# mwhittaker/frankenpaxos

Hardware: NVIDIA H100
Metric: committed slots/sec (simulated) at 1M in-flight slots (higher is better)
Workload: dtype int32

## Files before the change

frankenpaxos_b200/_lib.py:

```python
import ctypes as C
import os

from . import build as _build

_lib = None

SYMBOLS = [
    "fpx_abi_version", "fpx_strerror", "fpx_last_error", "fpx_create", "fpx_destroy", "fpx_reset",
    "fpx_proxyleader_arm", "fpx_acceptor_phase2a", "fpx_proxyleader_phase2b", "fpx_replica_chosen",
    "fpx_chosen_watermark", "fpx_quorum_eval", "fpx_snapshot_acceptor", "fpx_snapshot_log",
    "fpx_proxyleader_arm_dev", "fpx_acceptor_phase2a_dev", "fpx_proxyleader_phase2b_dev",
    "fpx_replica_chosen_dev", "fpx_replica_chosen_last_dev", "fpx_chosen_watermark_dev", "fpx_sync",
    "fpx_stream", "fpx_launch_count", "fpx_set_coop_ctas_per_sm", "fpx_step_dev", "fpx_step_kernel_ms", "fpx_step_arm_ms",
    "fpx_acceptor_phase1a", "fpx_leader_safe_values",
    "fpx_vm_client_request", "fpx_vm_phase2a", "fpx_vm_learn_chosen", "fpx_vm_skip", "fpx_vm_client_request_dev", "fpx_vm_phase2a_dev", "fpx_vm_step_dev",
    "fpx_mencius_arm_range", "fpx_mencius_acceptor_noop_range", "fpx_mencius_range_phase2b",
    "fpx_mencius_replica_chosen_range", "fpx_mencius_replica_range_first", "fpx_mencius_replica_range_fill",
    "fpx_wire_decode_inbound", "fpx_wire_decode_inbound_dev", "fpx_wire_encode_phase2b", "fpx_wire_encode_phase2b_dev",
    "fpx_wire_encode_nack", "fpx_wire_encode_chosen",
    "fpx_step_submit", "fpx_step_wait", "fpx_retire_below", "fpx_exchange_export", "fpx_exchange_attach", "fpx_exchange_attach_local", "fpx_exchange_epoch",
    "fpx_global_watermark", "fpx_global_watermark_dev",
    "fpx_conflict_index_create", "fpx_conflict_index_destroy", "fpx_conflict_index_put_snapshot", "fpx_conflict_index_batch",
    "fpx_depgraph_create", "fpx_depgraph_destroy", "fpx_depgraph_commit", "fpx_depgraph_update_executed", "fpx_depgraph_execute",
    "fpx_epaxos_stream", "fpx_epaxos_sync", "fpx_epaxos_lead_dev", "fpx_epaxos_preaccept_dev", "fpx_epaxos_accept_dev",
# ... 47 lines not shown
    L.fpx_snapshot_acceptor.restype = i32
    L.fpx_snapshot_log.argtypes = [vp, i32, i32, vp]; L.fpx_snapshot_log.restype = i32
    L.fpx_proxyleader_arm_dev.argtypes = [vp, vp, i32]; L.fpx_proxyleader_arm_dev.restype = i32
    L.fpx_acceptor_phase2a_dev.argtypes = [vp, vp, i32, vp, vp]; L.fpx_acceptor_phase2a_dev.restype = i32
    L.fpx_proxyleader_phase2b_dev.argtypes = [vp, vp, i32, vp]; L.fpx_proxyleader_phase2b_dev.restype = i32
    L.fpx_replica_chosen_dev.argtypes = [vp, vp, i32]; L.fpx_replica_chosen_dev.restype = i32
    L.fpx_replica_chosen_last_dev.argtypes = [vp, vp]; L.fpx_replica_chosen_last_dev.restype = i32
    L.fpx_chosen_watermark_dev.argtypes = [vp, vp]; L.fpx_chosen_watermark_dev.restype = i32
    L.fpx_acceptor_phase1a.argtypes = [vp, i32, i32, i32, p(i32)]; L.fpx_acceptor_phase1a.restype = i32
    L.fpx_leader_safe_values.argtypes = [vp, C.c_uint32, i32, i32, vp, vp, p(i32)]; L.fpx_leader_safe_values.restype = i32
    L.fpx_vm_client_request.argtypes = [vp, vp, i32, p(i64)]; L.fpx_vm_client_request.restype = i32
    L.fpx_vm_phase2a.argtypes = [vp, vp, i32, vp, p(i64)]; L.fpx_vm_phase2a.restype = i32
    L.fpx_vm_learn_chosen.argtypes = [vp, vp, i32, p(i64)]; L.fpx_vm_learn_chosen.restype = i32
    L.fpx_vm_skip.argtypes = [vp, vp, i32, p(i64)]; L.fpx_vm_skip.restype = i32
    L.fpx_vm_client_request_dev.argtypes = [vp, vp, i32]; L.fpx_vm_client_request_dev.restype = i32
    L.fpx_vm_phase2a_dev.argtypes = [vp, vp, i32, vp]; L.fpx_vm_phase2a_dev.restype = i32
    L.fpx_mencius_arm_range.argtypes = [vp, vp, i32, p(i64)]; L.fpx_mencius_arm_range.restype = i32
    L.fpx_mencius_acceptor_noop_range.argtypes = [vp, vp, i32, vp, p(i32), vp, p(i32), p(i64)]
    L.fpx_mencius_acceptor_noop_range.restype = i32
    L.fpx_mencius_range_phase2b.argtypes = [vp, vp, i32, vp, p(i32), p(i64)]; L.fpx_mencius_range_phase2b.restype = i32
    L.fpx_mencius_replica_chosen_range.argtypes = [vp, vp, i32, p(i64)]
    L.fpx_mencius_replica_chosen_range.restype = i32
    L.fpx_mencius_replica_range_first.argtypes = [vp, vp, i32, vp, p(i64)]; L.fpx_mencius_replica_range_first.restype = i32
    L.fpx_mencius_replica_range_fill.argtypes = [vp, vp, i32, vp, p(i64)]; L.fpx_mencius_replica_range_fill.restype = i32
    L.fpx_wire_decode_inbound.argtypes = [vp, i32, vp, vp, i32, vp, vp, p(i64)]; L.fpx_wire_decode_inbound.restype = i32
    L.fpx_wire_decode_inbound_dev.argtypes = [vp, i32, vp, vp, i32, vp, vp]; L.fpx_wire_decode_inbound_dev.restype = i32
    L.fpx_wire_encode_phase2b.argtypes = [vp, vp, i32, vp, i32, vp, p(i64)]; L.fpx_wire_encode_phase2b.restype = i32
    L.fpx_wire_encode_phase2b_dev.argtypes = [vp, vp, i32, vp, i32, vp]; L.fpx_wire_encode_phase2b_dev.restype = i32
    L.fpx_wire_encode_nack.argtypes = [vp, vp, i32, vp, i32, vp, p(i64)]; L.fpx_wire_encode_nack.restype = i32
    L.fpx_wire_encode_chosen.argtypes = [vp, vp, i32, vp, vp, i32, vp, i32, vp, p(i64)]
    L.fpx_wire_encode_chosen.restype = i32
    L.fpx_step_dev.argtypes = [vp, vp, i32, vp, i32, vp, vp, vp, i32, vp, vp, i32]; L.fpx_step_dev.restype = i32
    L.fpx_vm_step_dev.argtypes = [vp, vp, i32, vp, i32, vp, vp, i32, vp, vp]; L.fpx_vm_step_dev.restype = i32
    L.fpx_step_kernel_ms.argtypes = [vp, i32, p(C.c_float), p(C.c_float)]; L.fpx_step_kernel_ms.restype = i32
    L.fpx_step_arm_ms.argtypes = [vp, i32, p(C.c_float)]; L.fpx_step_arm_ms.restype = i32
    L.fpx_sync.argtypes = [vp, p(SyncResult)]; L.fpx_sync.restype = i32
    L.fpx_set_coop_ctas_per_sm.argtypes = [vp, i32]; L.fpx_set_coop_ctas_per_sm.restype = i32
    L.fpx_stream.argtypes = [vp]; L.fpx_stream.restype = vp
    L.fpx_launch_count.argtypes = [vp]; L.fpx_launch_count.restype = i64
    L.fpx_retire_below.argtypes = [vp, i32]; L.fpx_retire_below.restype = i32
    L.fpx_step_submit.argtypes = [vp, vp, i32, vp, i32, vp, i32, vp, vp, vp]; L.fpx_step_submit.restype = i32
    L.fpx_step_wait.argtypes = [vp, p(i32), p(i32), p(i32), p(i32), p(i64)]; L.fpx_step_wait.restype = i32
    L.fpx_exchange_export.argtypes = [vp, vp]; L.fpx_exchange_export.restype = i32
    L.fpx_exchange_attach.argtypes = [vp, i32, vp]; L.fpx_exchange_attach.restype = i32
    L.fpx_exchange_attach_local.argtypes = [vp, i32, vp]; L.fpx_exchange_attach_local.restype = i32
    L.fpx_exchange_epoch.argtypes = [vp]; L.fpx_exchange_epoch.restype = C.c_uint32
    L.fpx_global_watermark_dev.argtypes = [vp, C.c_uint32, i32, vp, vp]; L.fpx_global_watermark_dev.restype = i32
    L.fpx_global_watermark.argtypes = [vp, C.c_uint32, i32, p(i32), vp]; L.fpx_global_watermark.restype = i32
    if hasattr(L, "fpx_debug_set_tally_path"):
        L.fpx_debug_set_tally_path.argtypes = [vp, i32]; L.fpx_debug_set_tally_path.restype = i32
        L.fpx_debug_last_tally_path.argtypes = [vp]; L.fpx_debug_last_tally_path.restype = i32
    if hasattr(L, "fpx_debug_set_acceptor_segments"):
        L.fpx_debug_set_acceptor_segments.argtypes = [vp, i32]; L.fpx_debug_set_acceptor_segments.restype = i32
    if L.fpx_abi_version() != 1:
        raise ImportError("libfpx.so ABI version mismatch")
    _lib = L
    return L
```

frankenpaxos_b200/csrc/fpx_arm.cuh:

```cuda
#pragma once
#include "fpx_common.cuh"
#include "fpx_ranges.cuh"

namespace fpx {

struct ArmConflict { int32_t slot, round; };

struct ArmParams {
  Geometry g;
  PLState pl;
  const int4* in;
  int32_t n;
  DevStatus* st;
  ArmConflict* conflicts;
  uint32_t* win_bits;
  unsigned long long* votes;
  int32_t vanilla;
  RangeTable rng;
  int32_t check_rng;
};

__device__ __forceinline__ void note_arm_conflict(const ArmParams& P, int slot, int round) {
  uint32_t c = atomicAdd(&P.st->n_arm_conflicts, 1u);
  if (c < (uint32_t)kMaxConflicts) P.conflicts[c] = ArmConflict{slot, round};
}

__device__ __forceinline__ bool claim_header(const ArmParams& P, RowRef r, int slot, int round, int value,
                                             bool* other_round) {
  unsigned long long want = ((unsigned long long)(uint32_t)value << 32) | (uint32_t)round;
  unsigned long long old = atomicCAS(r.hdr64(), kU64Empty, want);
  *other_round = false;
  if (old == kU64Empty) return true;
  uint32_t orw = (uint32_t)old;
  if ((int)(orw & ~kDoneBit) != round) { *other_round = true; return false; }
  if ((uint32_t)(old >> 32) != (uint32_t)value) note_arm_conflict(P, slot, round);
  return false;
}

__device__ __forceinline__ uint32_t* table_insert(const ArmParams& P, int slot, int round) {
  const Geometry& g = P.g;
  if (g.ovf_cap == 0) return nullptr;
  unsigned long long key = ((unsigned long long)(uint32_t)slot << 32) | (uint32_t)round;
  uint32_t h = (uint32_t)mix64(key) & g.ovf_mask;
  for (int probe = 0; probe < g.ovf_cap; ++probe) {
    unsigned long long k = atomicCAS(&P.pl.ovf_keys[h], kU64Empty, key);
    if (k == kU64Empty || k == key) return P.pl.ovf_rows + (size_t)h * g.row_words;
    h = (h + 1) & g.ovf_mask;
  }
  return nullptr;
}

__device__ __forceinline__ bool arm_finish(const ArmParams& P, const int4& rec, unsigned long long old, int i) {
  const Geometry& g = P.g;
  const int slot = rec.x, round = rec.y, value = rec.z;
  if (old == kU64Empty) return true;
  uint32_t* prim = P.pl.rows + (size_t)local_slot(g, slot) * g.row_words;
  unsigned long long* hdr = (unsigned long long*)prim;
  while (true) {
    uint32_t orw = (uint32_t)old;
    if (orw == kBusy) {
      __nanosleep(64);
      old = *(volatile unsigned long long*)hdr;
      continue;
    }
    if (orw == kPoison) {
      uint32_t* t = table_insert(P, slot, round);
      if (t == nullptr) { report_error(P.st, FPX_ERR_OVERFLOW_FULL, i); return false; }
      bool dummy;
      return claim_header(P, RowRef{t}, slot, round, value, &dummy);
    }
    if ((int)(orw & ~kDoneBit) == round) {
      if ((uint32_t)(old >> 32) != (uint32_t)value) note_arm_conflict(P, slot, round);
      return false;
// ... 73 lines not shown
      if (local[u] >= 0 && old[u] != kU64Empty) {
        const int4 rec = __ldcg(P.in + i);
        won = arm_finish(P, rec, old[u], i);
        self = rec.w & 0xffff;
      } else if (won && P.vanilla) {
        self = rel_to_slot(g, ring_to_rel(g, local[u])) % g.per_group;
      }
      if (won && P.vanilla) {
        uint32_t* row = P.pl.rows + (size_t)local[u] * g.row_words;
        auto stamp = [&](int w) { return w - 2 == self ? 0u : kStampEmpty; };
        *(uint2*)(row + 2) = make_uint2(stamp(2), stamp(3));
        for (int w = 4; w < g.row_words; w += 4) *(uint4*)(row + w) = make_uint4(stamp(w), stamp(w + 1), stamp(w + 2), stamp(w + 3));
        red_max_u64(&P.votes[cell_index(g, local[u], self)], (((want[u] & 0xffffffffull) + 1ull) << 32) | (want[u] >> 32));
      }
      unsigned wb = __ballot_sync(0xffffffffu, won);
      if (lane == 0) P.win_bits[c0 + u] = wb;
      int ml = __reduce_max_sync(0xffffffffu, won ? local[u] : -1);
      if (lane == 0 && ml > max_local) max_local = ml;
    }
  }
  return max_local;
}

__device__ __forceinline__ void arm_resolve_conflicts(const ArmParams& P) {
  const Geometry& g = P.g;
  __shared__ int s_min, s_any;
  uint32_t nc = __ldcg(&P.st->n_arm_conflicts);
  if (nc == 0) return;
  if (nc > (uint32_t)kMaxConflicts) {
    if (threadIdx.x == 0) { report_error(P.st, FPX_ERR_CONFLICT, 0); P.st->n_arm_conflicts = 0; }
    return;
  }
  for (uint32_t c = 0; c < nc; ++c) {
    int slot = P.conflicts[c].slot, round = P.conflicts[c].round;
    if (threadIdx.x == 0) { s_min = INT_MAX; s_any = 0; }
    __syncthreads();
    for (int j = threadIdx.x; j < P.n; j += blockDim.x) {
      int4 rec = P.in[j];
      if (rec.x == slot && rec.y == round) {
        atomicMin(&s_min, j);
        if ((__ldcg(&P.win_bits[j >> 5]) >> (j & 31)) & 1u) s_any = 1;
      }
    }
    __syncthreads();
    if (threadIdx.x == 0 && s_any && s_min != INT_MAX) {
      RowRef r = find_row(g, P.pl, local_slot(g, slot), slot, round);
      if (r.p != nullptr) r.p[1] = (uint32_t)P.in[s_min].z;
    }
    __syncthreads();
  }
  if (threadIdx.x == 0) P.st->n_arm_conflicts = 0;
}

__global__ void __launch_bounds__(kArmThreads, 1) arm_kernel(ArmParams P) {
  const int lane = threadIdx.x & 31;
  const int max_local = arm_chunks(P, blockIdx.x * (blockDim.x >> 5) + (threadIdx.x >> 5), gridDim.x * (blockDim.x >> 5), lane);
  if (lane == 0 && max_local >= 0) atomicMax(&P.st->max_armed_local, max_local);

  __shared__ bool s_last;
  __syncthreads();
  if (threadIdx.x == 0) {
    __threadfence();
    s_last = (atomicAdd(&P.st->ticket, 1u) == gridDim.x - 1);
  }
  __syncthreads();
  if (!s_last) return;
  __threadfence();
  if (threadIdx.x == 0) P.st->ticket = 0;
  arm_resolve_conflicts(P);
}

}
```

frankenpaxos_b200/csrc/fpx_common.cuh:

```cuda
#pragma once
#include <cuda_runtime.h>
#include <stdint.h>

#include "../../include/fpx.h"

namespace fpx {

constexpr uint32_t kUnarmed = 0xffffffffu;
constexpr uint32_t kDoneBit = 0x80000000u;
constexpr uint32_t kPoison = 0xfffffffeu;
constexpr uint32_t kBusy = 0xfffffffdu;
constexpr uint32_t kStampEmpty = 0xffffffffu;
constexpr uint64_t kU64Empty = ~0ull;
constexpr uint64_t kCellChosen = 0x8000000000000000ull;
constexpr int kThreads = 256;
constexpr int kWarps = kThreads / 32;
constexpr int kMaxKeys = FPX_MAX_ACCEPTORS;
constexpr int kMaxConflicts = 1024;
constexpr int kSms = 132;
constexpr int kMaxGrid = kSms * 8;
constexpr uint32_t kTsBadVoter = 1u, kTsAnomaly = 2u, kTsPoison = 4u, kTsVanillaRound = 8u;

struct DevStatus {
  unsigned long long err_word;
  int32_t n_p2b, n_nack, n_chosen, watermark;
  uint32_t n_conflicts;
  uint32_t ticket;
  int32_t wm_local;
  int32_t max_chosen_local;
  int32_t wm_found;
  uint32_t bar_count;
  uint32_t nack_total;
  uint32_t pad[2];
  int32_t max_armed_local;
  uint32_t bar_gen;
  int32_t ts_min_local, ts_max_local;
  int32_t ts_min_round, ts_max_round;
  uint32_t ts_flags;
  uint32_t ts_path;
  uint32_t n_arm_conflicts;
  uint32_t wm_need_scan;
  unsigned long long t_acceptor[8];
  unsigned long long t_tally[8];
};

__device__ __forceinline__ unsigned long long global_timer_ns() {
  unsigned long long t;
  asm volatile("mov.u64 %0, %%globaltimer;" : "=l"(t));
  return t;
}
#define FPX_MARK(arr, k) do { if (blockIdx.x == 0 && threadIdx.x == 0) (arr)[k] = global_timer_ns(); } while (0)

constexpr int kMaxShards = 64;
struct DevExchange {
  int32_t enabled, n, mine, pad;
  uint32_t epoch;
  uint32_t pad2;
  unsigned long long* tabs[kMaxShards];
};
__device__ __forceinline__ void exchange_publish(DevExchange* x, int global_frontier) {
  if (x == nullptr || !x->enabled) return;
  const uint32_t ep = ++x->epoch;
  const unsigned long long v = ((unsigned long long)ep << 32) | (uint32_t)global_frontier;
  for (int p = 0; p < x->n; ++p)
    if (x->tabs[p] != nullptr)
      asm volatile("st.global.relaxed.sys.u64 [%0], %1;" ::"l"(x->tabs[p] + x->mine), "l"(v) : "memory");
}

struct Geometry {
  int32_t protocol, f, groups, per_group, flexible, num_leaders;
  int32_t voters;
  int32_t num_keys;
  int32_t quorum;
  int32_t row_words;
  int32_t slot_capacity;
  int32_t local_slots;
  int32_t base_local;
  int32_t base_ring;
  int32_t shard_index, shard_count;
  uint32_t ovf_mask;
  int32_t ovf_cap;
  unsigned long long m_groups, m_shards;
  int32_t cell_shift;
  int32_t lgroups, agroups;
  unsigned long long m_lgroups, m_agroups;
};

__device__ __forceinline__ uint32_t fastmod_u32(uint32_t a, unsigned long long M, uint32_t d) {
  unsigned long long low = M * a;
  return (uint32_t)__umul64hi(low, d);
}
__device__ __forceinline__ uint32_t fastdiv_u32(uint32_t a, unsigned long long M) {
  return (uint32_t)__umul64hi(M, a);
}

__device__ __forceinline__ int4 ld_stream(const int4* p) {
  int4 r;
  asm volatile("ld.global.nc.L1::no_allocate.v4.s32 {%0,%1,%2,%3}, [%4];"
               : "=r"(r.x), "=r"(r.y), "=r"(r.z), "=r"(r.w)
               : "l"(p));
  return r;
}
__device__ __forceinline__ unsigned long long l2_policy_evict_last() {
  unsigned long long pol;
  asm volatile("createpolicy.fractional.L2::evict_last.b64 %0, 1.0;" : "=l"(pol));
  return pol;
}
__device__ __forceinline__ unsigned long long l2_policy_evict_normal() {
  unsigned long long pol;
  asm volatile("createpolicy.fractional.L2::evict_normal.b64 %0, 1.0;" : "=l"(pol));
  return pol;
}
__device__ __forceinline__ unsigned long long l2_policy_evict_first() {
  unsigned long long pol;
  asm volatile("createpolicy.fractional.L2::evict_first.b64 %0, 1.0;" : "=l"(pol));
  return pol;
}
__device__ __forceinline__ void st_evict_first(int4* p, int4 v, unsigned long long pol) {
  asm volatile("st.global.L1::no_allocate.L2::cache_hint.v4.s32 [%0], {%1,%2,%3,%4}, %5;" ::"l"(p), "r"(v.x), "r"(v.y),
               "r"(v.z), "r"(v.w), "l"(pol));
}
__device__ __forceinline__ int4 ld_keep(const int4* p, unsigned long long pol) {
  int4 r;
  asm volatile("ld.global.nc.L1::no_allocate.L2::cache_hint.v4.s32 {%0,%1,%2,%3}, [%4], %5;"
               : "=r"(r.x), "=r"(r.y), "=r"(r.z), "=r"(r.w)
               : "l"(p), "l"(pol));
  return r;
}
__device__ __forceinline__ int4 ld_hint(const int4* p, unsigned long long pol) {
  int4 r;
  asm volatile("ld.global.L1::no_allocate.L2::cache_hint.v4.s32 {%0,%1,%2,%3}, [%4], %5;"
               : "=r"(r.x), "=r"(r.y), "=r"(r.z), "=r"(r.w)
               : "l"(p), "l"(pol));
  return r;
}
__device__ __forceinline__ unsigned long long ld_u64_evict_last(const unsigned long long* p) {
  unsigned long long v;
  asm volatile("{ .reg .b64 pol; createpolicy.fractional.L2::evict_last.b64 pol, 1.0; "
               "ld.global.cg.L2::cache_hint.u64 %0, [%1], pol; }"
               : "=l"(v) : "l"(p));
  return v;
}

__device__ __forceinline__ void red_min_u32(uint32_t* p, uint32_t v) {
  asm volatile("red.global.min.u32 [%0], %1;" ::"l"(p), "r"(v) : "memory");
}
__device__ __forceinline__ void red_or_u32(uint32_t* p, uint32_t v) {
  asm volatile("red.global.or.b32 [%0], %1;" ::"l"(p), "r"(v) : "memory");
}
__device__ __forceinline__ void red_min_u64(unsigned long long* p, unsigned long long v) {
  asm volatile("red.global.min.u64 [%0], %1;" ::"l"(p), "l"(v) : "memory");
}
__device__ __forceinline__ void red_max_u64(unsigned long long* p, unsigned long long v) {
  asm volatile("red.global.max.u64 [%0], %1;" ::"l"(p), "l"(v) : "memory");
}
__device__ __forceinline__ void st_stream(int4* p, int4 v) {
  asm volatile("st.global.L1::no_allocate.v4.s32 [%0], {%1,%2,%3,%4};" ::"l"(p), "r"(v.x), "r"(v.y),
               "r"(v.z), "r"(v.w));
}
__device__ __forceinline__ void st_stream2(int2* p, int2 v) {
  asm volatile("st.global.L1::no_allocate.v2.s32 [%0], {%1,%2};" ::"l"(p), "r"(v.x), "r"(v.y));
}
__device__ __forceinline__ unsigned lanemask_lt() {
  unsigned m;
  asm("mov.u32 %0, %%lanemask_lt;" : "=r"(m));
  return m;
}

__device__ __forceinline__ void report_error(DevStatus* st, int code, long long index) {
  unsigned long long w = ((unsigned long long)index << 8) | (unsigned long long)(unsigned)(-code);
  atomicMin(&st->err_word, w);
}

constexpr int kLocalRetired = -2;
__device__ __forceinline__ int local_slot(const Geometry& g, int slot) {
  if ((uint32_t)slot >= (uint32_t)g.slot_capacity) return -1;
  int u = slot;
  if (g.shard_count != 1) {
    uint32_t q = fastdiv_u32((uint32_t)slot, g.m_shards);
    if ((int)((uint32_t)slot - q * (uint32_t)g.shard_count) != g.shard_index) return -1;
    u = (int)q;
  }
  const int rel = u - g.base_local;
  if (rel < 0) return kLocalRetired;
  if (rel >= g.local_slots) return -1;
  const int ring = rel + g.base_ring;
  return ring >= g.local_slots ? ring - g.local_slots : ring;
}
__device__ __forceinline__ int ring_to_rel(const Geometry& g, int ring) {
  const int rel = ring - g.base_ring;
  return rel < 0 ? rel + g.local_slots : rel;
}
__device__ __forceinline__ int rel_to_ring(const Geometry& g, long long rel) {
  const long long r = rel + g.base_ring;
  return (int)(r >= g.local_slots ? r - g.local_slots : r);
// ... 119 lines not shown
```

frankenpaxos_b200/csrc/fpx_engine.cu:

```cuda
#include <cuda_runtime.h>
#include <stdio.h>
#include <stdlib.h>
#include <string.h>

#include <algorithm>
#include <new>
#include <string>
#include <vector>

#include "fpx_acceptor.cuh"
#include "fpx_arm.cuh"
#include "fpx_common.cuh"
#include "fpx_conflict.cuh"
#include "fpx_depgraph.cuh"
#include "fpx_epaxos.cuh"
#include "fpx_ranges.cuh"
#include "fpx_replica_misc.cuh"
#include "fpx_tally.cuh"
#include "fpx_vanilla.cuh"
#include "fpx_wire.cuh"

using namespace fpx;

constexpr int kMaxEvents = 16;
constexpr int kTallySmem = 200 * 1024 / (1024 / kTT);
constexpr int kStepRing = 1024;

struct fpx_engine {
  fpx_config cfg;
  Geometry g;
  cudaStream_t stream = nullptr;
  cudaStream_t h2d_stream = nullptr, d2h_stream = nullptr;
  cudaEvent_t ev[16] = {};
  uint32_t* rows = nullptr;
  unsigned long long* ovf_keys = nullptr;
  uint32_t* ovf_rows = nullptr;
  unsigned long long* votes = nullptr;
  int32_t* acc_round = nullptr;
  int32_t* acc_max_voted = nullptr;
  unsigned long long* rlog = nullptr;
  uint32_t vm_tag = 1;
  uint32_t* rng_tab = nullptr;
  int32_t rng_cap = 0;
  int32_t* rng_dec = nullptr;
  uint32_t rng_seq_base = 1;
  int unit_ranges = 0;
  cudaEvent_t* step_ev = nullptr;
  struct WireBuf { void* p = nullptr; size_t cap = 0; };
  WireBuf w_bytes, w_offs, w_kind, w_rec, w_out, w_tiles, w_arena, w_voffs;
  DevStatus* st = nullptr;
  DevExchange* xch = nullptr;
  DevExchange h_xch;
  unsigned long long* xch_table = nullptr;
  void* xch_opened[kMaxShards] = {};
  uint32_t xch_epoch = 0;
  int32_t* xch_out = nullptr;
  uint32_t* bits = nullptr;
  int32_t* g_agg = nullptr;
  uint32_t* g_wacc = nullptr;
  uint2* t_bw = nullptr;
  uint32_t* t_cc = nullptr;
  void* t_tmp = nullptr;
  int tally_path = 0;
  int acc_segments = 0;
  long long l2_bytes = 0;
  void* conflicts = nullptr;
  void* arm_conflicts = nullptr;
  uint32_t* arm_bits = nullptr;
  void* d_in = nullptr;
  void* d_out_a = nullptr;
  void* d_out_b = nullptr;
  DevStatus* h_st = nullptr;
  struct Lane {
    void *d_p2a = nullptr, *d_p2b = nullptr, *d_arm = nullptr, *d_out_p2b = nullptr, *d_out_nack = nullptr, *d_out_chosen = nullptr;
    cudaEvent_t ev_p2a = nullptr, ev_p2b = nullptr, ev_acc = nullptr, ev_done = nullptr, ev_d2h = nullptr;
    DevStatus* h_st = nullptr;
    fpx_p2b* out_p2b = nullptr; fpx_nack* out_nack = nullptr; fpx_chosen* out_chosen = nullptr;
    int32_t n_p2a = 0;
    bool busy = false;
  } lane[2];
  int lane_head = 0, lane_tail = 0, lanes_in_flight = 0;
  uint32_t parity = 0;
  int grid_acceptor = 0;
  int grid_tally = 0;
  int occ_acceptor = 0, occ_tally = 0;
  int tally_max_sub = 0;
  int num_sms = 0;
  uint32_t seq_base = 1;
  uint32_t rseq_base = 1;
  int32_t last_p2b_n = 0;
  int64_t launches = 0;
  std::string last_error;
};

#define CK(e, call)                                                              \
  do {                                                                           \
    cudaError_t _err = (call);                                                   \
    if (_err != cudaSuccess) {                                                   \
      (e)->last_error = std::string(#call) + ": " + cudaGetErrorString(_err);   \
      return FPX_ERR_CUDA;                                                       \
    }                                                                            \
  } while (0)

static int validate(const fpx_config* c) {
  if (c->f < 1) return FPX_ERR_CONFIG;
  if (c->num_leaders < c->f + 1) return FPX_ERR_CONFIG;
  if (c->num_replicas < c->f + 1) return FPX_ERR_CONFIG;
  if (c->num_acceptor_groups < 1 || c->acceptors_per_group < 1) return FPX_ERR_CONFIG;
  if (!c->flexible) {
    if (c->acceptors_per_group != 2 * c->f + 1) return FPX_ERR_CONFIG;
  } else {
    if (std::min(c->num_acceptor_groups, c->acceptors_per_group) - 1 < c->f) return FPX_ERR_CONFIG;
  }
  if (c->protocol != FPX_MULTIPAXOS && c->protocol != FPX_MENCIUS && c->protocol != FPX_VANILLA_MENCIUS)
    return FPX_ERR_UNSUPPORTED;
  if (c->protocol == FPX_VANILLA_MENCIUS && (c->flexible || c->num_acceptor_groups != 1)) return FPX_ERR_CONFIG;
  int lgroups = 1;
// ... 244 lines not shown
  if (e->h2d_stream) cudaStreamDestroy(e->h2d_stream);
  if (e->d2h_stream) cudaStreamDestroy(e->d2h_stream);
  if (e->stream) cudaStreamDestroy(e->stream);
  delete e;
}

int fpx_reset(fpx_engine* e) {
  if (!e) return FPX_ERR_INVALID_ARG;
  CK(e, cudaSetDevice(e->cfg.device));
  return reset_state(e);
}

void* fpx_stream(fpx_engine* e) { return e ? (void*)e->stream : nullptr; }

int fpx_retire_below(fpx_engine* e, int32_t slot) {
  if (!e || slot < 0) return FPX_ERR_INVALID_ARG;
  if (e->g.protocol == FPX_VANILLA_MENCIUS) return FPX_ERR_UNSUPPORTED;
  CK(e, cudaSetDevice(e->cfg.device));
  fpx_sync_result r;
  int c = fpx_sync(e, &r);
  if (c != FPX_OK) return c;
  if (slot > r.watermark) return FPX_ERR_INVALID_ARG;
  Geometry& g = e->g;
  long long new_base = ((long long)slot - g.shard_index + g.shard_count - 1) / g.shard_count;
  if (new_base < g.base_local) new_base = g.base_local;
  const int count = (int)std::min<long long>(new_base - g.base_local, g.local_slots);
  if (count == 0) return FPX_OK;
  recycle_kernel<<<std::min(count * 8 + 255, kSms * 2048) / 256 + 1, 256, 0, e->stream>>>(g, e->rows, e->votes, e->rlog, 0, count);
  e->launches++;
  CK(e, cudaGetLastError());
  g.base_local = (int32_t)new_base;
  g.base_ring = (int32_t)(new_base % g.local_slots);
  long long cap = (long long)e->cfg.slot_capacity + (long long)g.base_local * g.shard_count;
  g.slot_capacity = (int32_t)std::min<long long>(cap, 0x7fffffffll);
  return FPX_OK;
}

int fpx_set_coop_ctas_per_sm(fpx_engine* e, int32_t ctas_per_sm) {
  if (!e || ctas_per_sm < 0) return FPX_ERR_INVALID_ARG;
  int a = ctas_per_sm == 0 ? e->occ_acceptor : std::min(e->occ_acceptor, ctas_per_sm);
  int t = ctas_per_sm == 0 ? e->occ_tally : std::min(e->occ_tally, ctas_per_sm);
  e->grid_acceptor = std::min(a * e->num_sms, kMaxGrid);
  e->grid_tally = std::min(t * e->num_sms, kMaxGrid);
  return FPX_OK;
}

int fpx_debug_phase_times(fpx_engine* e, unsigned long long* acceptor8, unsigned long long* tally8) {
  if (!e) return FPX_ERR_INVALID_ARG;
  CK(e, cudaStreamSynchronize(e->stream));
  CK(e, cudaMemcpy(acceptor8, e->st->t_acceptor, 64, cudaMemcpyDeviceToHost));
  CK(e, cudaMemcpy(tally8, e->st->t_tally, 64, cudaMemcpyDeviceToHost));
  return FPX_OK;
}
int64_t fpx_launch_count(const fpx_engine* e) { return e ? e->launches : 0; }
int fpx_debug_set_tally_path(fpx_engine* e, int32_t path) {
  if (!e || (path & ~6)) return FPX_ERR_INVALID_ARG;
  e->tally_path = path;
  return FPX_OK;
}
int fpx_debug_set_acceptor_segments(fpx_engine* e, int32_t segments) {
  if (!e || segments < 0 || segments > kAccMaxSegments) return FPX_ERR_INVALID_ARG;
  e->acc_segments = segments;
  return FPX_OK;
}
int fpx_debug_last_tally_path(fpx_engine* e) {
  if (!e) return FPX_ERR_INVALID_ARG;
  uint32_t v = 0;
  CK(e, cudaStreamSynchronize(e->stream));
  CK(e, cudaMemcpy(&v, &e->st->ts_path, 4, cudaMemcpyDeviceToHost));
  return (int)v;
}


static int check_n(fpx_engine* e, const void* p, int32_t n) {
  if (!e || n < 0 || n > e->cfg.max_batch || (n > 0 && !p)) return FPX_ERR_INVALID_ARG;
  return FPX_OK;
}

static ArmParams arm_params(fpx_engine* e, const fpx_p2a* d_in, int32_t n, int vanilla) {
  ArmParams P;
  P.g = e->g;
  P.pl = PLState{e->rows, e->ovf_keys, e->ovf_rows};
  P.in = (const int4*)d_in;
  P.n = n;
  P.st = e->st;
  P.conflicts = (ArmConflict*)e->arm_conflicts;
  P.win_bits = e->arm_bits;
  P.votes = e->votes;
  P.vanilla = vanilla;
  P.rng = RangeTable{e->rng_tab, (uint32_t)e->rng_cap - 1u, e->rng_cap};
  P.check_rng = e->unit_ranges;
  return P;
}

static int arm_launch(fpx_engine* e, const fpx_p2a* d_in, int32_t n, int vanilla) {
  int c = check_n(e, d_in, n);
  if (c != FPX_OK || n == 0) return c;
  ArmParams P = arm_params(e, d_in, n, vanilla);
  int arm_blocks = std::min((n + kArmThreads * kArmUnroll - 1) / (kArmThreads * kArmUnroll), e->num_sms);
  arm_kernel<<<arm_blocks, kArmThreads, 0, e->stream>>>(P);
  e->launches++;
  CK(e, cudaGetLastError());
  return FPX_OK;
}

int fpx_proxyleader_arm_dev(fpx_engine* e, const fpx_p2a* d_in, int32_t n) {
  if (e && e->g.protocol == FPX_VANILLA_MENCIUS) return FPX_ERR_UNSUPPORTED;
  return arm_launch(e, d_in, n, 0);
}

static int acceptor_launch(fpx_engine* e, const fpx_p2a* d_in, int32_t n, fpx_p2b* d_out_p2b, fpx_nack* d_out_nack,
                           int append, cudaStream_t stream);

int fpx_acceptor_phase2a_dev(fpx_engine* e, const fpx_p2a* d_in, int32_t n, fpx_p2b* d_out_p2b,
                             fpx_nack* d_out_nack) {
  return acceptor_launch(e, d_in, n, d_out_p2b, d_out_nack, 0, e ? e->stream : nullptr);
}

static int acceptor_launch(fpx_engine* e, const fpx_p2a* d_in, int32_t n, fpx_p2b* d_out_p2b, fpx_nack* d_out_nack,
                           int append, cudaStream_t stream) {
  int c = check_n(e, d_in, n);
  if (c != FPX_OK) return c;
  if (n > 0 && (!d_out_p2b || !d_out_nack)) return FPX_ERR_INVALID_ARG;
  if (e->g.protocol == FPX_VANILLA_MENCIUS) return FPX_ERR_UNSUPPORTED;
  if (n == 0) {
    if (!append) CK(e, cudaMemsetAsync(&e->st->n_p2b, 0, 8, stream));
    return FPX_OK;
  }
  AcceptorParams P;
  P.g = e->g;
  P.in = (const int4*)d_in;
  P.n = n;
  P.out_p2b = (int4*)d_out_p2b;
  P.out_nack = (int2*)d_out_nack;
  P.votes = e->votes;
  P.acc_round = e->acc_round;
  P.acc_max_voted = e->acc_max_voted;
  P.accept_bits = e->bits;
  P.g_agg = e->g_agg;
  P.g_wacc = e->g_wacc;
  P.st = e->st;
  P.conflicts = (VoteConflict*)e->conflicts;
  int grid = std::max(1, std::min(e->grid_acceptor, (n + kAT - 1) / kAT));
  P.segments = e->acc_segments > 0 ? e->acc_segments : acceptor_segments(n, e->l2_bytes);
  P.parity = e->parity;
  P.append = append;
  e->parity ^= 1u;
  void* args[] = {&P};
  CK(e, cudaLaunchCooperativeKernel((const void*)acceptor_phase2a_kernel, dim3(grid), dim3(kAT), args,
                                    (size_t)(e->g.num_keys + P.segments) * kAT * 4, stream));
  e->launches++;
  CK(e, cudaGetLastError());
  return FPX_OK;
// ... 637 lines not shown
```

frankenpaxos_b200/engine.py:

```python
import ctypes as C

import numpy as np

from . import _lib

P2A = np.dtype([("slot", "<i4"), ("round", "<i4"), ("value_id", "<i4"), ("dst", "<i4")])
P2B = np.dtype([("group", "<i4"), ("acceptor", "<i4"), ("slot", "<i4"), ("round", "<i4")])
CHOSEN = np.dtype([("slot", "<i4"), ("value_id", "<i4")])
NACK = np.dtype([("leader", "<i4"), ("round", "<i4")])
P2A_RANGE = np.dtype([("slot_start", "<i4"), ("slot_end", "<i4"), ("round", "<i4"), ("dst", "<i4")])
P2B_RANGE = np.dtype([("dst", "<i4"), ("slot_start", "<i4"), ("slot_end", "<i4"), ("round", "<i4")])
CHOSEN_RANGE = np.dtype([("slot_start", "<i4"), ("slot_end", "<i4")])
VM_SKIP = np.dtype([("server", "<i4"), ("slot_start", "<i4"), ("slot_stop", "<i4"), ("own", "<i4")])
VALUE_NOOP = -(1 << 31)
WIRE_REC = np.dtype([("a", "<i4"), ("b", "<i4"), ("c", "<i4"), ("d", "<i4")])
WIRE_PROXYLEADER_INBOUND, WIRE_ACCEPTOR_INBOUND = 0, 1
WIRE_MENCIUS_PROXYLEADER_INBOUND, WIRE_MENCIUS_ACCEPTOR_INBOUND = 2, 3

MULTIPAXOS, MENCIUS, VANILLA_MENCIUS = 0, 1, 2

OK = 0
ERR_INVALID_ARG, ERR_CONFIG, ERR_CUDA, ERR_UNKNOWN_SLOT_ROUND, ERR_BAD_ACCEPTOR = -1, -2, -3, -4, -5
ERR_SLOT_RANGE, ERR_ROUND_RANGE, ERR_OVERFLOW_FULL, ERR_CONFLICT, ERR_NO_DEVICE, ERR_UNSUPPORTED = \
    -6, -7, -8, -9, -10, -11
# ... 55 lines not shown
        return self

    def __exit__(self, *a):
        self.close()

    def reset(self):
        self._check(self._L.fpx_reset(self.h))

    def retire_below(self, slot):
        self._check(self._L.fpx_retire_below(self.h, slot))

    def _check(self, st, idx=-1):
        if st != OK:
            detail = self._L.fpx_last_error(self.h).decode() if st == ERR_CUDA else ""
            raise FpxError(st, idx, detail)

    @property
    def stream(self):
        return self._L.fpx_stream(self.h)

    @property
    def launch_count(self):
        return self._L.fpx_launch_count(self.h)

    def exchange_export(self):
        buf = C.create_string_buffer(64)
        self._check(self._L.fpx_exchange_export(self.h, buf))
        return buf.raw

    def exchange_attach(self, shard, handle):
        self._check(self._L.fpx_exchange_attach(self.h, shard, C.c_char_p(bytes(handle))))

    def exchange_attach_local(self, shard, peer):
        self._check(self._L.fpx_exchange_attach_local(self.h, shard, peer.h))

    @property
    def exchange_epoch(self):
        return self._L.fpx_exchange_epoch(self.h)

    def global_watermark(self, epoch=None, timeout_ms=5000):
        n = self.cfg.shard_count
        fr = np.empty(n, dtype=np.int32)
        out = C.c_int32(0)
        ep = self.exchange_epoch if epoch is None else epoch
        self._check(self._L.fpx_global_watermark(self.h, ep, timeout_ms, C.byref(out), fr.ctypes.data))
        return out.value, fr

    def set_tally_path(self, exact):
        self._check(self._L.fpx_debug_set_tally_path(self.h, 2 if exact else 0))

    def set_acceptor_segments(self, segments):
        self._check(self._L.fpx_debug_set_acceptor_segments(self.h, segments))

    @property
    def last_tally_path(self):
        return {1: "sweep", 2: "exact"}.get(self._L.fpx_debug_last_tally_path(self.h), "none")

    def proxyleader_arm(self, p2a):
        p2a = np.ascontiguousarray(p2a, dtype=P2A)
        err = C.c_int64(-1)
        st = self._L.fpx_proxyleader_arm(self.h, p2a.ctypes.data, len(p2a), C.byref(err))
        self._check(st, err.value)

    def acceptor_phase2a(self, p2a):
        p2a = np.ascontiguousarray(p2a, dtype=P2A)
        n = len(p2a)
        out = np.empty(max(n, 1), dtype=P2B)
        nack = np.empty(max(n, 1), dtype=NACK)
        n1, n2, err = C.c_int32(0), C.c_int32(0), C.c_int64(-1)
        st = self._L.fpx_acceptor_phase2a(self.h, p2a.ctypes.data, n, out.ctypes.data, C.byref(n1),
                                          nack.ctypes.data, C.byref(n2), C.byref(err))
        self._check(st, err.value)
        return out[:n1.value], nack[:n2.value]

    def proxyleader_phase2b(self, p2b):
        p2b = np.ascontiguousarray(p2b, dtype=P2B)
        n = len(p2b)
        out = np.empty(max(n, 1), dtype=CHOSEN)
        n1, err = C.c_int32(0), C.c_int64(-1)
        st = self._L.fpx_proxyleader_phase2b(self.h, p2b.ctypes.data, n, out.ctypes.data, C.byref(n1),
                                             C.byref(err))
        self._check(st, err.value)
        return out[:n1.value]

    def replica_chosen(self, chosen):
        chosen = np.ascontiguousarray(chosen, dtype=CHOSEN)
        err = C.c_int64(-1)
        st = self._L.fpx_replica_chosen(self.h, chosen.ctypes.data, len(chosen), C.byref(err))
        self._check(st, err.value)

    def chosen_watermark(self):
        out = C.c_int32(0)
        self._check(self._L.fpx_chosen_watermark(self.h, C.byref(out)))
        return out.value

    def quorum_eval(self, which, masks):
        masks = np.ascontiguousarray(masks, dtype=np.uint32)
        out = np.empty(max(len(masks), 1), dtype=np.uint8)
        self._check(self._L.fpx_quorum_eval(self.h, which, masks.ctypes.data, len(masks), out.ctypes.data))
        return out[:len(masks)]

    def snapshot_acceptor(self, group, acceptor, first_slot=0, n_slots=0):
        vr = np.empty(max(n_slots, 1), dtype=np.int32)
        vv = np.empty(max(n_slots, 1), dtype=np.int32)
        r, m = C.c_int32(0), C.c_int32(0)
        self._check(self._L.fpx_snapshot_acceptor(self.h, group, acceptor, C.byref(r), C.byref(m), first_slot,
# ... 201 lines not shown
```

profiles/exp_step.py:

```python
import argparse
import ctypes
import json
import os
import sys

import numpy as np
import torch

ROOT = os.path.dirname(os.path.dirname(os.path.abspath(__file__)))
sys.path.insert(0, ROOT)
ap = argparse.ArgumentParser()
ap.add_argument("--steps", type=int, default=12)
ap.add_argument("--variants", default="default,acc_first,exact,default,acc_first")
ap.add_argument("--out", default="")
ap.add_argument("--old-lib", action="store_true", help="time the round-1 build (profiles/_r1/libfpx.so) instead")
ap.add_argument("--lib", default="", help="time another build of libfpx.so (tuning variants under profiles/_var/)")
args = ap.parse_args()
if args.old_lib:
    os.environ["FPX_LIB_OVERRIDE"] = os.path.join(ROOT, "profiles", "_r1", "libfpx.so")
if args.lib:
    os.environ["FPX_LIB_OVERRIDE"] = os.path.join(ROOT, args.lib)

import bench
from frankenpaxos_b200 import Engine, traces as T

cfg = bench.CFG
n = 1 << 20
S = args.steps + 3
dev = torch.device("cuda")


def td(x):
    return torch.from_numpy(x.view(np.int32).reshape(len(x), -1)).to(dev)


base = [T.workload(b, cfg, n) for b in range(4)]
outp = torch.empty((3 * n, 4), dtype=torch.int32, device=dev)
outn = torch.empty((3 * n, 2), dtype=torch.int32, device=dev)
outc = torch.empty((3 * n, 2), dtype=torch.int32, device=dev)
wm = torch.zeros(1, dtype=torch.int32, device=dev)
results = {}
for variant in args.variants.split(","):
    eng = Engine(slot_capacity=S * n, max_batch=3 * n, overflow_capacity=1 << 10, **cfg)
    L = eng._L
    L.fpx_debug_phase_times.argtypes = [ctypes.c_void_p, ctypes.c_void_p, ctypes.c_void_p]
    ext = torch.cuda.ExternalStream(eng.stream, device=dev)
    if not args.old_lib:
        eng._check(L.fpx_debug_set_tally_path(eng.h, sum(bit for tok, bit in (("exact", 2), ("nored", 4)) if tok in variant.split("_"))))
    for tok in variant.split("_"):
        if tok.startswith("seg"):
            eng.set_acceptor_segments(int(tok[3:]))
    flush = torch.empty(1 << 28, dtype=torch.uint8, device=dev) if "flush" in variant else None
    ins = []
    for s in range(S):
        a, p, b = base[s % 4]
        def rb(r):
            o = r.copy(); o["slot"] = o["slot"] + s * n; return o
        ins.append((td(rb(a)), td(rb(p)), td(rb(b))))
    torch.cuda.synchronize()
    names = ["arm", "acceptor", "tally", "replica", "watermark"]
    order = ["acceptor", "arm", "tally", "replica", "watermark"] if "accfirst" in variant.split("_") else names
    evs = [[torch.cuda.Event(enable_timing=True) for _ in range(6)] for _ in range(S)]

    def run(which, s):
        da, dp, db = ins[s]
        if which == "arm": eng.proxyleader_arm_dev(da.data_ptr(), n)
        elif which == "acceptor": eng.acceptor_phase2a_dev(dp.data_ptr(), 3 * n, outp.data_ptr(), outn.data_ptr())
        elif which == "tally":
            if flush is not None:
                with torch.cuda.stream(ext):
                    flush.view(torch.int64).sum()
                evs[s][order.index("tally")].record(ext)
            eng.proxyleader_phase2b_dev(db.data_ptr(), 3 * n, outc.data_ptr())
        elif which == "replica": eng.replica_chosen_last_dev(outc.data_ptr())
        else: eng.chosen_watermark_dev(wm.data_ptr())

    fused = "step" in variant.split("_")
    noev = "noev" in variant.split("_")
    import time
    t_host0 = time.perf_counter()
    for s in range(S):
        if s == 3 or not noev:
            evs[s][0].record(ext)
        if fused and noev:
            da, dp, db = ins[s]
            eng.step_dev(da.data_ptr(), n, dp.data_ptr(), 3 * n, outp.data_ptr(), outn.data_ptr(), db.data_ptr(), 3 * n,
                         outc.data_ptr(), wm.data_ptr(), ring_slot=-1)
            if s == S - 1:
                evs[s][5].record(ext)
            continue
        if fused:
            da, dp, db = ins[s]
            eng.step_dev(da.data_ptr(), n, dp.data_ptr(), 3 * n, outp.data_ptr(), outn.data_ptr(), db.data_ptr(), 3 * n,
                         outc.data_ptr(), wm.data_ptr(), ring_slot=s)
            for j in range(5):
                evs[s][j + 1].record(ext)
            continue
        for j, which in enumerate(order):
            run(which, s)
            evs[s][j + 1].record(ext)
    t_host = (time.perf_counter() - t_host0) / S * 1e6
    r = eng.sync()
    if "nored" not in variant:
        assert r.status == 0 and r.n_chosen == n and r.watermark == S * n, (r.status, r.n_chosen, r.watermark)
    step = evs[3][0].elapsed_time(evs[S - 1][5]) * 1e3 / (S - 3)
    per = {} if noev else {which: float(np.mean([evs[s][j].elapsed_time(evs[s][j + 1]) for s in range(3, S)])) * 1e3
                           for j, which in enumerate(order)}
    if noev:
        per = {}
    elif fused:
        ms = np.array([eng.step_kernel_ms(s) for s in range(3, S)])
        per = {"acceptor": float(ms[:, 0].mean()) * 1e3, "tally+replica+wm": float(ms[:, 1].mean()) * 1e3}
        per["arm"] = step - sum(per.values())
    ta = (ctypes.c_ulonglong * 8)(); tt = (ctypes.c_ulonglong * 8)()
    L.fpx_debug_phase_times(eng.h, ta, tt)
    tt = np.array(tt[:8], dtype=np.int64)
    ta = np.array(ta[:6], dtype=np.int64)
    res = {"step_us": step, "host_enqueue_us_per_step": t_host, "kernels_us": per, "sum_kernels_us": sum(per.values()),
           "tally_path": "r1" if args.old_lib else eng.last_tally_path,
           "tally_phases_us(A,bar,B,bar,C,bar,D)": (np.diff(tt) / 1e3).round(1).tolist(),
           "acceptor_phases_us(p1,bar,carry,p2,bar)": (np.diff(ta) / 1e3).round(1).tolist()}
    print(variant, json.dumps(res), flush=True)
    results.setdefault(variant, []).append(res)
    eng.close()
    del ins
    torch.cuda.empty_cache()
if args.out:
    json.dump(results, open(args.out, "w"), indent=1)
```

Baseline: 3.514 billion.

## Add ordered non-atomic arm fast path with cooperative grid sync

```diff
diff --git a/frankenpaxos_b200/_lib.py b/frankenpaxos_b200/_lib.py
--- a/frankenpaxos_b200/_lib.py
+++ b/frankenpaxos_b200/_lib.py
@@ -123,6 +123,10 @@
         L.fpx_debug_last_tally_path.argtypes = [vp]; L.fpx_debug_last_tally_path.restype = i32
     if hasattr(L, "fpx_debug_set_acceptor_segments"):
         L.fpx_debug_set_acceptor_segments.argtypes = [vp, i32]; L.fpx_debug_set_acceptor_segments.restype = i32
+    if hasattr(L, "fpx_debug_set_store_paths"):
+        L.fpx_debug_set_store_paths.argtypes = [vp, i32]; L.fpx_debug_set_store_paths.restype = i32
+        L.fpx_debug_last_store_paths.argtypes = [vp]; L.fpx_debug_last_store_paths.restype = i32
+        L.fpx_debug_arm_phase_times.argtypes = [vp, vp]; L.fpx_debug_arm_phase_times.restype = i32
     if L.fpx_abi_version() != 1:
         raise ImportError("libfpx.so ABI version mismatch")
     _lib = L
diff --git a/frankenpaxos_b200/csrc/fpx_arm.cuh b/frankenpaxos_b200/csrc/fpx_arm.cuh
--- a/frankenpaxos_b200/csrc/fpx_arm.cuh
+++ b/frankenpaxos_b200/csrc/fpx_arm.cuh
@@ -18,7 +18,28 @@
   int32_t vanilla;
   RangeTable rng;
   int32_t check_rng;
+  int32_t try_ordered;
 };
+
+template <bool kRanges = true>
+__device__ __forceinline__ int arm_record_row(const ArmParams& P, const int4& rec, int i) {
+  const Geometry& g = P.g;
+  const int l = local_slot(g, rec.x);
+  if (l < 0) {
+    if (l != kLocalRetired) report_error(P.st, FPX_ERR_SLOT_RANGE, i);
+  } else if ((uint32_t)rec.y > (uint32_t)FPX_MAX_ROUND) {
+    report_error(P.st, FPX_ERR_ROUND_RANGE, i);
+  } else if (P.vanilla && rec.y != 0) {
+    report_error(P.st, FPX_ERR_ROUND_RANGE, i);
+  } else if (P.vanilla && ((rec.w >> 16) != 0 || (rec.w & 0xffff) >= g.per_group ||
+                           rec.x % g.per_group != (rec.w & 0xffff))) {
+    report_error(P.st, FPX_ERR_BAD_ACCEPTOR, i);
+  } else if (kRanges && P.check_rng && range_find(P.rng, rec.x, rec.x + 1, rec.y) != nullptr) {
+  } else {
+    return l;
+  }
+  return -1;
+}
 
 __device__ __forceinline__ void note_arm_conflict(const ArmParams& P, int slot, int round) {
   uint32_t c = atomicAdd(&P.st->n_arm_conflicts, 1u);
@@ -198,22 +219,151 @@
   if (threadIdx.x == 0) P.st->n_arm_conflicts = 0;
 }
 
+__device__ __forceinline__ bool arm_check_order(const ArmParams& P, int lo, int hi, int lane) {
+  const unsigned full = 0xffffffffu;
+  bool ok = true;
+  int ps = 0, pr = 0;
+  if (lo > 0 && lo < hi) { const int4 b = __ldcg(P.in + lo - 1); ps = b.x; pr = b.y; }
+  for (int c0 = lo; c0 < hi; c0 += 32 * kArmUnroll) {
+    int4 rec[kArmUnroll];
+#pragma unroll
+    for (int u = 0; u < kArmUnroll; ++u) {
+      const int i = c0 + u * 32 + lane;
+      rec[u] = i < hi ? ld_stream(P.in + i) : make_int4(-1, 0, 0, 0);
+    }
+#pragma unroll
+    for (int u = 0; u < kArmUnroll; ++u) {
+      if (c0 + u * 32 >= hi) break;
+      const int i = c0 + u * 32 + lane;
+      int s_up = __shfl_up_sync(full, rec[u].x, 1), r_up = __shfl_up_sync(full, rec[u].y, 1);
+      if (lane == 0) { s_up = ps; r_up = pr; }
+      ps = __shfl_sync(full, rec[u].x, 31);
+      pr = __shfl_sync(full, rec[u].y, 31);
+      if (i < hi) {
+        arm_record_row<false>(P, rec[u], i);
+        if (i > 0 && (rec[u].x < s_up || (rec[u].x == s_up && rec[u].y != r_up))) ok = false;
+      }
+    }
+  }
+  return __all_sync(full, ok);
+}
+
+constexpr int kArmOrderedUnroll = 4;
+
+__device__ __forceinline__ int arm_ordered(const ArmParams& P, int lo, int hi, int lane) {
+  const Geometry& g = P.g;
+  const unsigned full = 0xffffffffu;
+  int max_local = -1;
+  int ps = lo > 0 && lo < hi ? __ldcg(&P.in[lo - 1].x) : 0;
+  for (int c0 = lo; c0 < hi; c0 += 32 * kArmOrderedUnroll) {
+    unsigned long long old[kArmOrderedUnroll];
+    unsigned long long want[kArmOrderedUnroll];
+    int local[kArmOrderedUnroll];
+    {
+      int4 rec[kArmOrderedUnroll];
+#pragma unroll
+      for (int u = 0; u < kArmOrderedUnroll; ++u) {
+        const int i = c0 + u * 32 + lane;
+        rec[u] = i < hi ? ld_last_use(P.in + i) : make_int4(-1, 0, 0, 0);
+      }
+#pragma unroll
+      for (int u = 0; u < kArmOrderedUnroll; ++u) {
+        const int i = c0 + u * 32 + lane;
+        int s_up = __shfl_up_sync(full, rec[u].x, 1);
+        if (lane == 0) s_up = ps;
+        ps = __shfl_sync(full, rec[u].x, 31);
+        local[u] = -1;
+        old[u] = 0;
+        if (i < hi && (i == 0 || rec[u].x != s_up)) {
+          const int l = arm_record_row<false>(P, rec[u], i);
+          if (l >= 0) {
+            local[u] = l;
+            want[u] = ((unsigned long long)(uint32_t)rec[u].z << 32) | (uint32_t)rec[u].y;
+            old[u] = ld_u64_evict_last((const unsigned long long*)(P.pl.rows + (size_t)l * g.row_words));
+          }
+        }
+      }
+    }
+    unsigned stored = 0, slow = 0;
+#pragma unroll
+    for (int u = 0; u < kArmOrderedUnroll; ++u) {
+      if (local[u] < 0) continue;
+      if (old[u] == kU64Empty) {
+        st_u64_evict_last((unsigned long long*)(P.pl.rows + (size_t)local[u] * g.row_words), want[u]);
+        stored |= 1u << u;
+      } else {
+        slow |= 1u << u;
+      }
+    }
+#pragma unroll
+    for (int u = 0; u < kArmOrderedUnroll; ++u) {
+      if (c0 + u * 32 >= hi) break;
+      const int i = c0 + u * 32 + lane;
+      bool won = (stored >> u) & 1u;
+      if ((slow >> u) & 1u) {
+        const unsigned long long* hdr = (const unsigned long long*)(P.pl.rows + (size_t)local[u] * g.row_words);
+        won = arm_finish(P, __ldcg(P.in + i), __ldcg(hdr), i);
+      }
+      const unsigned wb = __ballot_sync(full, won);
+      if (lane == 0) P.win_bits[(c0 + u * 32) >> 5] = wb;
+      const int ml = __reduce_max_sync(full, won ? local[u] : -1);
+      if (ml > max_local) max_local = ml;
+    }
+  }
+  return max_local;
+}
+
+__device__ __forceinline__ void arm_warp_range(int n, int& lo, int& hi) {
+  const int total_warps = gridDim.x * (kArmThreads / 32), gw = blockIdx.x * (kArmThreads / 32) + (threadIdx.x >> 5);
+  const int per = (((n + total_warps - 1) / total_warps) + 31) & ~31;
+  lo = (int)min((long long)n, (long long)gw * per);
+  hi = min(n, lo + per);
+}
+
+__device__ __forceinline__ void arm_mark(const ArmParams& P, int k) {
+  if (blockIdx.x == 0 && threadIdx.x == 0) {
+    unsigned long long* t = P.st->t_arm;
+    asm volatile("" : "+l"(t));
+    t[k] = global_timer_ns();
+  }
+}
+
 __global__ void __launch_bounds__(kArmThreads, 1) arm_kernel(ArmParams P) {
   const int lane = threadIdx.x & 31;
-  const int max_local = arm_chunks(P, blockIdx.x * (blockDim.x >> 5) + (threadIdx.x >> 5), gridDim.x * (blockDim.x >> 5), lane);
+  int lo, hi;
+  bool ordered = false;
+  if (P.try_ordered) {
+    arm_mark(P, 0);
+    arm_warp_range(P.n, lo, hi);
+    if (!arm_check_order(P, lo, hi, lane) && lane == 0) atomicOr(&P.st->arm_unordered, 1u);
+    arm_mark(P, 1);
+    grid_sync(P.st);
+    arm_mark(P, 2);
+    ordered = __ldcg(&P.st->arm_unordered) == 0;
+  } else {
+    arm_mark(P, 0);
+    arm_mark(P, 1);
+    arm_mark(P, 2);
+  }
+  int max_local;
+  if (!ordered) {
+    max_local = arm_chunks(P, blockIdx.x * (kArmThreads / 32) + (threadIdx.x >> 5), gridDim.x * (kArmThreads / 32), lane);
+  } else {
+    arm_warp_range(P.n, lo, hi);
+    max_local = arm_ordered(P, lo, hi, lane);
+  }
   if (lane == 0 && max_local >= 0) atomicMax(&P.st->max_armed_local, max_local);
-
-  __shared__ bool s_last;
-  __syncthreads();
+  arm_mark(P, 3);
+
+  grid_sync(P.st);
+  arm_mark(P, 4);
+  if (blockIdx.x != 0) return;
   if (threadIdx.x == 0) {
-    __threadfence();
-    s_last = (atomicAdd(&P.st->ticket, 1u) == gridDim.x - 1);
-  }
-  __syncthreads();
-  if (!s_last) return;
-  __threadfence();
-  if (threadIdx.x == 0) P.st->ticket = 0;
+    P.st->arm_path = P.try_ordered && __ldcg(&P.st->arm_unordered) == 0 ? 1u : 0u;
+    P.st->arm_unordered = 0;
+  }
   arm_resolve_conflicts(P);
-}
-
-}
+  arm_mark(P, 5);
+}
+
+}
diff --git a/frankenpaxos_b200/csrc/fpx_common.cuh b/frankenpaxos_b200/csrc/fpx_common.cuh
--- a/frankenpaxos_b200/csrc/fpx_common.cuh
+++ b/frankenpaxos_b200/csrc/fpx_common.cuh
@@ -42,6 +42,9 @@
   uint32_t wm_need_scan;
   unsigned long long t_acceptor[8];
   unsigned long long t_tally[8];
+  unsigned long long t_arm[8];
+  uint32_t arm_unordered;
+  uint32_t arm_path;
 };
 
 __device__ __forceinline__ unsigned long long global_timer_ns() {
@@ -141,6 +144,19 @@
                : "=l"(v) : "l"(p));
   return v;
 }
+__device__ __forceinline__ void st_u64_evict_last(unsigned long long* p, unsigned long long v) {
+  asm volatile("{ .reg .b64 pol; createpolicy.fractional.L2::evict_last.b64 pol, 1.0; "
+               "st.global.L2::cache_hint.u64 [%0], %1, pol; }"
+               :: "l"(p), "l"(v) : "memory");
+}
+__device__ __forceinline__ int4 ld_last_use(const int4* p) {
+  int4 r;
+  asm volatile("{ .reg .b64 pol; createpolicy.fractional.L2::evict_first.b64 pol, 1.0; "
+               "ld.global.L1::no_allocate.L2::cache_hint.v4.s32 {%0,%1,%2,%3}, [%4], pol; }"
+               : "=r"(r.x), "=r"(r.y), "=r"(r.z), "=r"(r.w)
+               : "l"(p));
+  return r;
+}
 
 __device__ __forceinline__ void red_min_u32(uint32_t* p, uint32_t v) {
   asm volatile("red.global.min.u32 [%0], %1;" ::"l"(p), "r"(v) : "memory");
diff --git a/frankenpaxos_b200/csrc/fpx_engine.cu b/frankenpaxos_b200/csrc/fpx_engine.cu
--- a/frankenpaxos_b200/csrc/fpx_engine.cu
+++ b/frankenpaxos_b200/csrc/fpx_engine.cu
@@ -25,6 +25,7 @@
 constexpr int kMaxEvents = 16;
 constexpr int kTallySmem = 200 * 1024 / (1024 / kTT);
 constexpr int kStepRing = 1024;
+constexpr int kForceAtomicArm = 1;
 
 struct fpx_engine {
   fpx_config cfg;
@@ -63,6 +64,7 @@
   void* t_tmp = nullptr;
   int tally_path = 0;
   int acc_segments = 0;
+  int store_force = 0;
   long long l2_bytes = 0;
   void* conflicts = nullptr;
   void* arm_conflicts = nullptr;
@@ -413,6 +415,12 @@
   CK(e, cudaMemcpy(tally8, e->st->t_tally, 64, cudaMemcpyDeviceToHost));
   return FPX_OK;
 }
+int fpx_debug_arm_phase_times(fpx_engine* e, unsigned long long* arm8) {
+  if (!e) return FPX_ERR_INVALID_ARG;
+  CK(e, cudaStreamSynchronize(e->stream));
+  CK(e, cudaMemcpy(arm8, e->st->t_arm, 64, cudaMemcpyDeviceToHost));
+  return FPX_OK;
+}
 int64_t fpx_launch_count(const fpx_engine* e) { return e ? e->launches : 0; }
 int fpx_debug_set_tally_path(fpx_engine* e, int32_t path) {
   if (!e || (path & ~6)) return FPX_ERR_INVALID_ARG;
@@ -423,6 +431,18 @@
   if (!e || segments < 0 || segments > kAccMaxSegments) return FPX_ERR_INVALID_ARG;
   e->acc_segments = segments;
   return FPX_OK;
+}
+int fpx_debug_set_store_paths(fpx_engine* e, int32_t mask) {
+  if (!e || (mask & ~kForceAtomicArm)) return FPX_ERR_INVALID_ARG;
+  e->store_force = mask;
+  return FPX_OK;
+}
+int fpx_debug_last_store_paths(fpx_engine* e) {
+  if (!e) return FPX_ERR_INVALID_ARG;
+  uint32_t v = 0;
+  CK(e, cudaStreamSynchronize(e->stream));
+  CK(e, cudaMemcpy(&v, &e->st->arm_path, 4, cudaMemcpyDeviceToHost));
+  return (int)v;
 }
 int fpx_debug_last_tally_path(fpx_engine* e) {
   if (!e) return FPX_ERR_INVALID_ARG;
@@ -451,6 +471,7 @@
   P.vanilla = vanilla;
   P.rng = RangeTable{e->rng_tab, (uint32_t)e->rng_cap - 1u, e->rng_cap};
   P.check_rng = e->unit_ranges;
+  P.try_ordered = !vanilla && !e->unit_ranges && !(e->store_force & kForceAtomicArm);
   return P;
 }
 
@@ -459,7 +480,8 @@
   if (c != FPX_OK || n == 0) return c;
   ArmParams P = arm_params(e, d_in, n, vanilla);
   int arm_blocks = std::min((n + kArmThreads * kArmUnroll - 1) / (kArmThreads * kArmUnroll), e->num_sms);
-  arm_kernel<<<arm_blocks, kArmThreads, 0, e->stream>>>(P);
+  void* args[] = {&P};
+  CK(e, cudaLaunchCooperativeKernel((const void*)arm_kernel, dim3(arm_blocks), dim3(kArmThreads), args, 0, e->stream));
   e->launches++;
   CK(e, cudaGetLastError());
   return FPX_OK;
diff --git a/frankenpaxos_b200/engine.py b/frankenpaxos_b200/engine.py
--- a/frankenpaxos_b200/engine.py
+++ b/frankenpaxos_b200/engine.py
@@ -131,6 +131,16 @@
     def set_acceptor_segments(self, segments):
         self._check(self._L.fpx_debug_set_acceptor_segments(self.h, segments))
 
+    def set_store_paths(self, atomic_arm=False):
+        self._check(self._L.fpx_debug_set_store_paths(self.h, 1 if atomic_arm else 0))
+
+    @property
+    def last_store_paths(self):
+        v = self._L.fpx_debug_last_store_paths(self.h)
+        if v < 0:
+            self._check(v)
+        return {"arm": "ordered" if v & 1 else "atomic"}
+
     @property
     def last_tally_path(self):
         return {1: "sweep", 2: "exact"}.get(self._L.fpx_debug_last_tally_path(self.h), "none")
diff --git a/profiles/exp_step.py b/profiles/exp_step.py
--- a/profiles/exp_step.py
+++ b/profiles/exp_step.py
@@ -50,6 +50,8 @@
     for tok in variant.split("_"):
         if tok.startswith("seg"):
             eng.set_acceptor_segments(int(tok[3:]))
+    if hasattr(L, "fpx_debug_set_store_paths"):
+        eng.set_store_paths(atomic_arm="atomarm" in variant.split("_"))
     flush = torch.empty(1 << 28, dtype=torch.uint8, device=dev) if "flush" in variant else None
     ins = []
     for s in range(S):
@@ -111,15 +113,26 @@
     elif fused:
         ms = np.array([eng.step_kernel_ms(s) for s in range(3, S)])
         per = {"acceptor": float(ms[:, 0].mean()) * 1e3, "tally+replica+wm": float(ms[:, 1].mean()) * 1e3}
-        per["arm"] = step - sum(per.values())
+        per["arm+gaps"] = step - sum(per.values())
+        arm_kernel = float(np.mean([eng.step_arm_ms(s) for s in range(3, S)])) * 1e3
     ta = (ctypes.c_ulonglong * 8)(); tt = (ctypes.c_ulonglong * 8)()
     L.fpx_debug_phase_times(eng.h, ta, tt)
     tt = np.array(tt[:8], dtype=np.int64)
     ta = np.array(ta[:6], dtype=np.int64)
+    arm_ph = []
+    if not fused or noev:
+        arm_kernel = None
+    if hasattr(L, "fpx_debug_arm_phase_times"):
+        tarm = (ctypes.c_ulonglong * 8)()
+        L.fpx_debug_arm_phase_times(eng.h, tarm)
+        arm_ph = (np.diff(np.array(tarm[:6], dtype=np.int64)) / 1e3).round(1).tolist()
     res = {"step_us": step, "host_enqueue_us_per_step": t_host, "kernels_us": per, "sum_kernels_us": sum(per.values()),
+           "arm_kernel_us(events)": arm_kernel,
            "tally_path": "r1" if args.old_lib else eng.last_tally_path,
            "tally_phases_us(A,bar,B,bar,C,bar,D)": (np.diff(tt) / 1e3).round(1).tolist(),
-           "acceptor_phases_us(p1,bar,carry,p2,bar)": (np.diff(ta) / 1e3).round(1).tolist()}
+           "acceptor_phases_us(p1,bar,carry,p2,bar)": (np.diff(ta) / 1e3).round(1).tolist(),
+           "arm_phases_us(check,bar,arms,bar,resolve)": arm_ph,
+           "store_paths": eng.last_store_paths if hasattr(L, "fpx_debug_last_store_paths") else None}
     print(variant, json.dumps(res), flush=True)
     results.setdefault(variant, []).append(res)
     eng.close()
```

Measured after the change: 3.582 billion, median of 6. 1.9% higher.
